# zeahmed/NeuralASR

Measured on AMD Instinct MI355X. Metric: audio-frames/sec (fwd+bwd+CTC+Adam) at batch 16 per GPU, higher is better.
Workload: dtype f32

## Files before the change

neuralasr_amd/csrc/nasr_api.hip:

```cpp
#include "nasr_ctx.h"

using namespace nasr;
using namespace nasr_impl;

namespace {
int settle_end(nasr_ctx* h, nasr_ctx::StepEnd& e, int* void_out) {
  if (!wait_stamp(e.stamp, e.seq, 60.0)) return h->fail(NASR_ERR_HIP, "nasr_settle_step: the step did not end within 60 s");
  if (*e.host != 0.f) {
    *void_out = 1;
    (void)rec_check(h);
  }
  return NASR_OK;
}
}

namespace nasr_impl {

int create_fail(nasr_ctx* h, int code, const std::string& m) {
  g_create_error = m;
  nasr_destroy(h);
  return code;
}

int handle_open(const char* fn, Family family, int device_id, void* stream, nasr_ctx** out, hipDeviceProp_t* prop) {
// ... 162 lines not shown
      for (int i = 0; i < h->ndense; ++i) {
        h->off_dftp[i] = df; df += tph_bytes(h->dWp[i], h->dIp[i]);
        h->off_dbtp[i] = db; if (i > 0 || h->npre == 0) db += tph_bytes(h->dIp[i], h->dWp[i]);
      }
      if (hipMalloc(h->WfTP.out(), of) != hipSuccess ||
          hipMalloc(h->WbTP.out(), std::max<size_t>(ob, 1024)) != hipSuccess ||
          hipMalloc(h->DfTP.out(), std::max<size_t>(df, 1024)) != hipSuccess ||
          hipMalloc(h->DbTP.out(), std::max<size_t>(db, 1024)) != hipSuccess)
        return create_fail(h, NASR_ERR_HIP, "hipMalloc of the tiled weight planes failed");
    }
  }
  const size_t ub = (size_t)h->L * h->D * h->Hp * h->N4 * 4;
  if (!alloc_param_buffers(h) || hipMalloc(h->Uf.out(), ub) != hipSuccess || hipMalloc(h->Ub.out(), ub) != hipSuccess)
    return create_fail(h, NASR_ERR_HIP, "hipMalloc of parameter buffers failed");
  {
    h->bucket_of_layer.assign(h->L, -1);
    if (h->L > 1 && h->L <= MAX_BUCKETS) {
      for (int l = h->L - 1; l >= 1; --l) {
        const int64_t lo = h->off_wx[l], hi = l == h->L - 1 ? h->np_int : h->off_wx[l + 1];
        h->bucket_of_layer[l] = (int)h->buckets.size();
        h->buckets.push_back({GRAD_HEAD + lo, hi - lo});
      }
      h->buckets.push_back({0, GRAD_HEAD + h->off_wx[1]});
    } else if (h->L == 1 && h->npre > 0) {
      h->bucket_of_layer[0] = 0;
      h->buckets.push_back({GRAD_HEAD + h->off_wx[0], h->np_int - h->off_wx[0]});
      h->buckets.push_back({0, GRAD_HEAD + h->off_wx[0]});
    } else {
      h->buckets.push_back({0, GRAD_HEAD + h->np_int});
    }
  }
  (void)hipMemsetAsync(h->Uf, 0, ub, h->st);
  (void)hipMemsetAsync(h->Ub, 0, ub, h->st);
  {
    const char* e = getenv("NASR_PERSIST");
    const char* er = getenv("NASR_REC");
    if (rec_setup(h, !(e && e[0] == '0') && prop.multiProcessorCount == 256, er && std::string(er) == "f32") != NASR_OK)
      return create_fail(h, NASR_ERR_HIP, t_err);
  }
  h->gates.resize(h->L);
  h->OTT.resize(h->L);
  h->ott_valid.assign(h->L, 0);
  h->outb.resize(h->L);
  h->cbuf.resize(h->L);
  h->Ybuf.resize(h->ndense);
  h->dYbuf.resize(h->ndense);
  if (int rc = handle_finish(h)) return rc;
  {
    const char* eo = getenv("NASR_WGRAD_OVERLAP");
    const bool eligible = h->rec_kind == RecKind::Persist && h->Hp == 512 && h->L > 1;
    h->wg_overlap = eligible && !(eo && eo[0] == '0');
    h->ev_wg.resize(h->L);
    h->wg_pending.assign(h->L, 0);
    if (eligible) {
      int lo = 0, hi = 0;
      (void)hipDeviceGetStreamPriorityRange(&lo, &hi);
      if (hipStreamCreateWithPriority(h->wst.out(), hipStreamNonBlocking, lo) != hipSuccess ||
          hipEventCreateWithFlags(h->ev_dx.out(), hipEventDisableTiming) != hipSuccess)
        return create_fail(h, NASR_ERR_HIP, "set-up of the weight-gradient side stream failed");
      for (auto& e : h->ev_wg)
        if (hipEventCreateWithFlags(e.out(), hipEventDisableTiming) != hipSuccess) return create_fail(h, NASR_ERR_HIP, "hipEventCreate failed");
      h->bwd_lean = true;
    }
  }
  if (h->rec_kind != RecKind::Step) {
    const char* er = getenv("NASR_PERSIST_REARM");
    h->rearm_after = er && *er ? std::max<long long>(0, atoll(er)) : 200;
  }
  if (h->rec_kind == RecKind::Persist) {
    const char* eb = getenv("NASR_BUCKET_DEFER");
    h->bucket_defer = !(eb && eb[0] == '0');
  }
  rec_start(h);
  *out = h;
  return NASR_OK;
}

int nasr_destroy(nasr_handle h) {
  if (!h) return NASR_OK;
  (void)hipSetDevice(h->device);
  for (const Stream* s : {&h->st, &h->cst, &h->d2h, &h->wst})
    if (*s) (void)hipStreamSynchronize(*s);
  (void)nasr_comm_destroy(h);
  drop_graphs(h);
  delete h;
  return NASR_OK;
}

const char* nasr_last_error(nasr_handle h) {
  if (!h) return g_create_error.c_str();
  return t_err_handle == h ? t_err.c_str() : "";
}
const char* nasr_backend(nasr_handle) { return "hip-gfx950"; }

int nasr_synchronize(nasr_handle h) {
  if (!h) return NASR_ERR_ARG;
  return sync_checked(h);
}

int64_t nasr_param_count(nasr_handle h) {
  MODEL_CALL(h);
  return h ? h->np_tf : -1;
}
int nasr_num_tensors(nasr_handle h) {
  MODEL_CALL(h);
  return h ? (int)h->tensors.size() : -1;
}

int nasr_tensor_info(nasr_handle h, int idx, char name[64], int64_t* offset, int64_t* rows, int64_t* cols) {
  MODEL_CALL(h);
  if (!h) return NASR_ERR_ARG;
  if (idx < 0 || idx >= (int)h->tensors.size()) return h->fail(NASR_ERR_ARG, "tensor index out of range");
  const TensorInfo& t = h->tensors[idx];
  if (name) {
    strncpy(name, t.name.c_str(), 63);
// ... 741 lines not shown
int nasr_get_phase_times(nasr_handle h, nasr_phase_times* out) {
  MODEL_CALL(h);
  if (!h || !out) return NASR_ERR_ARG;
  HIPCHK(h, hipStreamSynchronize(h->st));
  float acc[PH_COUNT] = {0};
  for (const auto& s : h->spans) {
    float ms = 0.f;
    if (hipEventElapsedTime(&ms, s.a, s.b) == hipSuccess) acc[s.ph] += ms;
  }
  nasr_phase_times t;
  memset(&t, 0, sizeof(t));
  t.pack_ms = acc[PH_PACK]; t.xproj_ms = acc[PH_XPROJ]; t.rec_fwd_ms = acc[PH_RECF]; t.proj_ctc_ms = acc[PH_PROJCTC];
  t.proj_bwd_ms = acc[PH_PROJB]; t.rec_bwd_ms = acc[PH_RECB]; t.wgrad_ms = acc[PH_WGRAD]; t.adam_ms = acc[PH_ADAM];
  float tot = 0.f;
  if (h->total_valid && hipEventElapsedTime(&tot, h->ev_total_a, h->ev_total_b) == hipSuccess) t.total_ms = tot;
  (void)hipGetLastError();
  t.rec_fwd_launches = h->n_fwd_launch;
  t.rec_bwd_launches = h->n_bwd_launch;
  *out = t;
  return NASR_OK;
}

int nasr_set_graph_mode(nasr_handle h, int enabled) {
  MODEL_CALL(h);
  if (!h) return NASR_ERR_ARG;
  h->graph_mode = enabled != 0;
  if (!h->graph_mode) drop_graphs(h);
  return NASR_OK;
}

int nasr_set_dropout_state(nasr_handle h, uint32_t seed, uint32_t counter) {
  MODEL_CALL(h);
  if (!h) return NASR_ERR_ARG;
  LSTM_CALL(h, "has no dropout");
  h->drop_seed = seed;
  h->drop_counter = counter;
  return NASR_OK;
}

int nasr_get_dropout_state(nasr_handle h, uint32_t* seed, uint32_t* counter) {
  MODEL_CALL(h);
  if (!h) return NASR_ERR_ARG;
  LSTM_CALL(h, "has no dropout");
  if (seed) *seed = h->drop_seed;
  if (counter) *counter = h->drop_counter;
  return NASR_OK;
}

int nasr_set_wgrad_overlap(nasr_handle h, int enabled) {
  MODEL_CALL(h);
  if (!h) return NASR_ERR_ARG;
  LSTM_CALL(h, "has no recurrence");
  if (enabled && !h->wst) return h->fail(NASR_ERR_STATE, "the weight-gradient side stream was not set up for this handle "
                                                         "(needs the persistent recurrence at Hp = 512 and more than one layer)");
  HIPCHK(h, hipStreamSynchronize(h->st));
  h->wg_overlap = enabled != 0;
  if (h->resident) return ensure_shape(h, h->B, h->T, h->Lmax);
  return NASR_OK;
}

int nasr_get_wgrad_overlap(nasr_handle h) {
  MODEL_CALL(h);
  return h && h->wg_overlap ? 1 : 0;
}

int nasr_set_bucket_defer(nasr_handle h, int defer) {
  MODEL_CALL(h);
  if (!h) return NASR_ERR_ARG;
  h->bucket_defer = defer != 0;
  return NASR_OK;
}

int nasr_get_persist_stats(nasr_handle h, int* aborts, int* rearms) {
  MODEL_CALL(h);
  if (!h) return NASR_ERR_ARG;
  if (aborts) *aborts = h->persist_aborts;
  if (rearms) *rearms = h->persist_rearms;
  return NASR_OK;
}

}
```

neuralasr_amd/csrc/nasr_batch.hip:

```cpp
#include "nasr_ctx.h"

using namespace nasr;
using namespace nasr_impl;

namespace nasr_impl {

int ensure_ctc_buffers(nasr_ctx* h, int B, int Bp, int T, int Tp, int Lmax, bool* grew) {
  const int KS = std::max(1, (2 * std::max(Lmax, 0) + 1 + 63) / 64);
  if (KS > 16) return h->fail(NASR_ERR_ARG, "label length > 511 not supported by the CTC lattice kernel");
  const int KSa = KS <= 1 ? 2 : KS <= 8 ? KS : (KS <= 12 ? 12 : 16);
  bool ok = true;
  ok &= h->logits.ensure((size_t)Tp * Bp * h->Cp * 4, grew);
  ok &= h->logz.ensure((size_t)Tp * Bp * 4, grew);
  ok &= h->alpha.ensure((size_t)B * (T + 8) * KSa * 64 * 4, grew);
  ok &= h->beta.ensure((size_t)B * (T + 8) * KSa * 64 * 4, grew);
  ok &= h->aoff.ensure((size_t)B * (T + 8) * 8, grew);
  ok &= h->boff.ensure((size_t)B * (T + 8) * 8, grew);
  ok &= h->logp.ensure((size_t)Bp * 8, grew);
  ok &= h->ctcprobs.ensure((size_t)Tp * Bp * h->Cp * 4, grew);
  ok &= h->ctckexp.ensure((size_t)B * 2 * ((T + 8) / 4 + 3) * 8, grew);
  ok &= h->nll.ensure((size_t)Bp * 4, grew);
  ok &= h->loss.ensure(16, grew);
  ok &= h->amax.ensure((size_t)Tp * Bp * 4, grew);
  ok &= h->ids.ensure((size_t)B * Tp * 4, grew);
// ... 13 lines not shown
  const size_t R = (size_t)T * Bp;
  const int D = h->D, Hp = h->Hp, N4 = h->N4;
  bool grew = false;
  bool ok = true;
  const int KSa = ensure_ctc_buffers(h, B, Bp, T, Tp, Lmax, &grew);
  if (KSa < 0) return KSa;
  ok &= h->X0.ensure(R * h->Fp * 4, &grew);
  ok &= h->seqbuf.ensure((size_t)Bp * 4, &grew);
  ok &= h->dout.ensure(R * D * Hp * 4, &grew);
  ok &= h->hstate.ensure((size_t)2 * D * Bp * Hp * 4, &grew);
  ok &= h->partial.ensure((size_t)2 * D * (Hp / 32) * Bp * Hp * 4, &grew);
  ok &= h->dcstate.ensure((size_t)2 * D * Bp * Hp * 4, &grew);
  ok &= h->dgbuf.ensure(R * D * N4 * 4, &grew);
  if (h->rec_kind == RecKind::Persist) ok &= h->dgmax.ensure(persist_dgmax_floats(T, Bp, Hp, D) * 4, &grew);
  {
    int ipmax = h->Fp, wmax = D * N4;
    for (int l = 0; l < h->L; ++l) ipmax = std::max(ipmax, h->Ip[l]);
    for (int i = 0; i < h->ndense; ++i) { ipmax = std::max(ipmax, h->dIp[i]); wmax = std::max(wmax, h->dWp[i]); }
    ok &= h->XTP.ensure(tph_bytes((int)R, ipmax), &grew);
    ok &= h->X0TTP.ensure(tph_bytes(h->Ip[0], (int)R), &grew);
    for (int l = 0; l < h->L; ++l) ok &= h->OTT[l].ensure(tph_bytes(D * Hp, (int)R), &grew);
    ok &= h->GTP.ensure(tph_bytes((int)R, wmax), &grew);
    ok &= h->GTTP.ensure(tph_bytes(wmax, (int)R), &grew);
    if (h->wg_overlap) {
      ok &= h->GTTP2.ensure(tph_bytes(wmax, (int)R), &grew);
      ok &= h->sc_gc2.ensure((size_t)wmax);
    }
    if (h->ndense) ok &= h->DTP.ensure(tph_bytes(ipmax, (int)R), &grew);
    {
      const size_t n15 = std::max<size_t>(R, (size_t)std::max(ipmax, wmax));
      if (n15 > h->sc15_n) {
        ok &= h->sc15.ensure(n15);
        if (ok) {
          launch_fill(h->sc15.sp(), 32768.f, (int)n15, h->st);
          launch_fill(h->sc15.ip(), 1.f / 32768.f, (int)n15, h->st);
          h->sc15_n = n15;
        }
      }
      ok &= h->sc_x0r.ensure(R) && h->sc_x0c.ensure((size_t)h->Fp);
      ok &= h->sc_gr.ensure(R) && h->sc_gc.ensure((size_t)wmax);
      if (h->compactable) {
        ok &= h->sc_cr.ensure(R + 64) && h->sc_cx.ensure(R + 64);
        ok &= h->OTS.ensure((h->wg_overlap ? 2 : 1) * tph_bytes(D * Hp, (int)R), &grew);
      }
      for (int i = 0; i < h->ndense; ++i) ok &= h->sc_yr[i].ensure(R) && h->sc_yc[i].ensure((size_t)h->dWp[i]);
      bool g2 = false;
      ok &= h->scws.ensure(tph_scale_ws_floats((int)R, std::max(ipmax, wmax)) * 4, &g2);
    }
  }
  int csw = std::max(D * N4, h->Cp);
  for (int i = 0; i < h->ndense; ++i) csw = std::max(csw, h->dWp[i]);
  ok &= h->csws.ensure((size_t)std::max(32, tp_split2_parts((int)R)) * csw * 4, &grew);
  if (h->wg_overlap) ok &= h->csws2.ensure((size_t)std::max(32, tp_split2_parts((int)R)) * csw * 4, &grew);
  for (int i = 0; i < h->ndense; ++i) {
    ok &= h->Ybuf[i].ensure(R * h->dWp[i] * 4, &grew);
    ok &= h->dYbuf[i].ensure(R * h->dWp[i] * 4, &grew);
  }
  for (int l = 0; l < h->L; ++l) {
    ok &= h->gates[l].ensure(R * D * N4 * 4, &grew);
    ok &= h->outb[l].ensure(R * D * Hp * 4, &grew);
    ok &= h->cbuf[l].ensure(R * D * Hp * 4, &grew);
  }
  if (!ok) return h->fail(NASR_ERR_HIP, "hipMalloc failed while sizing batch buffers");
  if (grew || Bp != h->Bp) drop_graphs(h);
  h->B = B; h->Bp = Bp; h->T = T; h->Lmax = Lmax; h->Tp = Tp; h->KS = KSa;
  return NASR_OK;
}

int validate_batch(nasr_ctx* h, const int32_t* seq_len, const int32_t* labels, const int32_t* label_len, int B, int T,
                   int Lmax, int num_classes) {
  const bool las = !num_classes && h->family == Family::Las;
  const int C = num_classes ? num_classes : h->C;
  if (B < 1 || B > 64) return h->fail(NASR_ERR_ARG, "per-GPU batch must be in [1,64]");
  if (T < 1) return h->fail(NASR_ERR_ARG, "T must be >= 1");
  for (int b = 0; b < B; ++b) {
    if (seq_len[b] < 1 || seq_len[b] > T)
      return h->fail(NASR_ERR_ARG, "seq_len[" + std::to_string(b) + "] out of [1,T]");
    if (!labels) continue;
    if (las) {
      if (label_len[b] < 0 || label_len[b] > Lmax)
        return h->fail(NASR_ERR_ARG, "label_len[" + std::to_string(b) + "] out of [0,Lmax]");
      for (int i = 0; i < Lmax; ++i) {
        const int v = labels[(size_t)b * Lmax + i];
        if (v < 0 || v >= C) return h->fail(NASR_ERR_ARG, "label id out of [0, num_classes-1]");
      }
      continue;
    }
    const int L = label_len[b];
    if (L < 0 || L > Lmax) return h->fail(NASR_ERR_ARG, "label_len[" + std::to_string(b) + "] out of [0,Lmax]");
    int rep = 0;
    for (int i = 0; i < L; ++i) {
      const int v = labels[(size_t)b * Lmax + i];
      if (v < 0 || v >= C - 1)
        return h->fail(NASR_ERR_ARG, "label id out of [0, num_classes-2] (blank = num_classes-1 is not a label)");
      if (i > 0 && v == labels[(size_t)b * Lmax + i - 1]) ++rep;
    }
    if (L + rep > seq_len[b])
      return h->fail(NASR_ERR_INFEASIBLE, "Not enough time for target transition sequence (required: " +
                                              std::to_string(L + rep) + ", available: " + std::to_string(seq_len[b]) +
                                              ") in sequence " + std::to_string(b));
  }
  return NASR_OK;
}

int validate_chunk(nasr_ctx* h, const int32_t* n_frames, int S, int Tc) {
  if (Tc < 1) return h->fail(NASR_ERR_ARG, "a stream chunk needs Tc >= 1");
// ... 306 lines not shown
```

neuralasr_amd/csrc/nasr_ctx.h:

```cpp
#pragma once
#include <hip/hip_runtime.h>

#include <dlfcn.h>
#include <sched.h>
#include <unistd.h>

#include <chrono>

#include <algorithm>
#include <cmath>
#include <cstdio>
#include <cstdlib>
#include <cstring>
#include <functional>
#include <map>
#include <memory>
#include <mutex>
#include <string>
#include <vector>

#include "../../include/nasr.h"
#include "kernels.h"
#include "resample.h"
#include "wave_aug.h"
// ... 250 lines not shown
  DevBuf scws;
  int gttp_layer = -1;
  int dgmax_layer = -1;
  DevBuf dgmax;
  DevPtr<float> Gbase;
  std::vector<std::pair<int64_t, int64_t>> buckets;
  std::vector<Event> ev_bucket;
  std::vector<int> bucket_of_layer;
  bool bucket_defer = true;
  DevPtr<AdamDev> adam_dev;
  float lr;
  float max_grad_norm = 0.f;
  DevPtr<ClipDev> clip_dev;
  DevPtr<double> clip_part;
  struct StepRes { Pinned<void> host; size_t cap = 0; Pinned<uint32_t> stamp; uint32_t seq = 0; bool valid = false; int B = 0, Bp = 0, Tp = 0; bool logits = false, greedy = false;
                   Event ev_lg; };
  StepRes res[2];
  int res_cur = 0;
  struct StepEnd { Pinned<float> host; uint32_t* stamp = nullptr; uint32_t seq = 0; bool valid = false; int64_t token = 0; };
  static constexpr int NEND = 4;
  StepEnd endw[NEND];
  int end_cur = 0;
  int64_t step_token = 0;
  uint32_t stamp_seq = 0;

  bool resident = false, have_grads = false, have_fwd = false;
  int B = 0, Bp = 0, T = 0, Lmax = 0, Tp = 0, KS = 1;
  int64_t frames = 0;
  std::vector<int32_t> h_seq;
  BatchSlot slots[NSLOT];
  BatchSlot* cur = nullptr;
  Stream cst;
  Stream d2h;
  Event ev_snap;
  DevBuf logits_snap;
  std::mutex slot_mu;
  int slot_rr = 0;
  int32_t *seq_p = nullptr, *lablen_p = nullptr, *labels_p = nullptr, *cstart_p = nullptr, *cpos_p = nullptr,
          *rowmap_p = nullptr;
  bool compactable = false;
  int cmp_rows = 0, cmp_rows_p = 0;
  int32_t *vrow_p = nullptr, *vprev_p = nullptr, *vnext_p = nullptr;
  SV sc_cr, sc_cx;
  DevBuf OTS;

  bool wg_overlap = false;
  bool bwd_lean = false;
  Stream wst;
  Event ev_dx;
  std::vector<Event> ev_wg;
  std::vector<char> wg_pending;
  DevBuf GTTP2, csws2, slabs2;
  SV sc_gc2;
  DevBuf XTP, X0TTP, GTP, GTTP;
  std::vector<DevBuf> OTT;
  std::vector<char> ott_valid;
  DevBuf ctcprobs, ctckexp;
  DevBuf seqbuf, X0, logits, logz, alpha, beta, aoff, boff, logp, nll, loss, slabs, csws, amax, ids, lens,
      stage;
  DevBuf al_logz, al_bp, al_path, al_score, al_logits, al_meta;
  std::vector<DevBuf> gates, outb, cbuf;
  DevBuf dout, hstate, partial, dcstate, dgbuf;

  bool graph_mode = true;
  bool step_decode = false, step_logits = false, have_decoded = false;
  bool step_greedy = false;
  std::map<GraphKey, hipGraphExec_t> graphs;

  bool profiling = false;
  std::vector<Event> ev_pool;
  size_t ev_used = 0;
  struct Span { int ph; hipEvent_t a, b; };
  std::vector<Span> spans;
  Event ev_total_a, ev_total_b;
  bool window_open = false, total_valid = false;
  int n_fwd_launch = 0, n_bwd_launch = 0;
  nasr_phase_times last_times;

  int fail(int code, const std::string& m) {
    t_err = m;
    t_err_handle = this;
    return code;
  }
};

namespace nasr_impl {

#define HIPCHK(h, expr)                                                                                   \
  do {                                                                                                    \
    hipError_t e_ = (expr);                                                                               \
    if (e_ != hipSuccess)                                                                                 \
      return (h)->fail(NASR_ERR_HIP, std::string(#expr) + ": " + hipGetErrorString(e_));                  \
  } while (0)
#define MODEL_CALL(h)                                                                                     \
  do {                                                                                                    \
    if ((h) && (h)->family == Family::Featurizer)                                                         \
      return (h)->fail(NASR_ERR_STATE, std::string(__func__) + ": a featurizer handle has no model");     \
  } while (0)
#define LSTM_CALL(h, reason)                                                                              \
  do {                                                                                                    \
    if ((h) && (h)->family != Family::Lstm)                                                               \
      return (h)->fail(NASR_ERR_STATE, std::string(__func__) + ": a WaveNet or LAS handle " reason);      \
  } while (0)
#define FAMILY_CALL(h, state, text)                                                                       \
  do {                                                                                                    \
    if (!(h)) return NASR_ERR_ARG;                                                                        \
// ... 118 lines not shown
  bool rs = false;
  int n = 0;
  std::vector<int64_t> uoff, foff;
  int64_t S_in = 0;
  size_t mb = 0, meta_bytes = 0, rmeta_bytes = 0;
  bool wave = false;
  WavePlan wp;
};
int fz_plan(nasr_ctx* eh, FzState& z, const std::string& fn, const int64_t* offsets, const int32_t* rates, int n, FzPlan* p);
int fz_wave_plan(nasr_ctx* eh, FzState& z, const std::string& fn, const nasr_wave_aug* wave, FzPlan* p);
size_t fz_stage_bytes(const FzPlan& p);
int fz_produce_slot(nasr_ctx* eh, nasr_ctx* fzh, const FzPlan& p, const float* audio, int Tb, float* dcentre, float* dpad,
                    void* pinned, hipStream_t st);
int fz_feature_width(const nasr_ctx* fzh, int* numcontext, int* frame_width);
int fz_static_width(const nasr_ctx* fzh);

struct FzFeedSlot {
  int64_t seg_off, ntail, in_off, nnew;
  int64_t keep_off, nkeep;
  int64_t lead;
  int64_t f_off, nfb, want;
  int64_t nnorm, upto, y_off;
  int64_t T;
  int64_t rows0, nrows;
  int64_t n_after;
};
struct FzFeedPlan {
  std::vector<FzFeedSlot> slot;
  int64_t seg_total = 0, in_total = 0, f_total = 0, y_total = 0;
  int Tc = 0;
};
int fz_stream_attach(nasr_ctx* eh, nasr_ctx* fzh, int S, std::unique_ptr<FzStream, FzStreamDelete>* out);
int fz_stream_plan(nasr_ctx* eh, const FzStream& a, const std::string& fn, const int64_t* nnew, const uint8_t* last, FzFeedPlan* p);
int fz_stream_run(nasr_ctx* eh, FzStream& a, const FzFeedPlan& p, const float* audio, float* dfeats, hipStream_t st);
void fz_stream_advance(FzStream& a, const FzFeedPlan& p, const uint8_t* last);
void fz_stream_reset(FzStream& a, int slot);

inline float* dout_of(nasr_ctx* h, int) { return h->dout.as<float>(); }
inline float* dg_of(nasr_ctx* h, int) { return h->dgbuf.as<float>(); }
inline bool wg_alt(const nasr_ctx* h, int l) { return h->wg_overlap && (l & 1); }
inline unsigned char* gttp_of(nasr_ctx* h, int l) { return (wg_alt(h, l) ? h->GTTP2 : h->GTTP).as<unsigned char>(); }
inline float* csws_of(nasr_ctx* h, int l) { return (wg_alt(h, l) ? h->csws2 : h->csws).as<float>(); }
inline nasr_ctx::SV& gc_of(nasr_ctx* h, int l) { return wg_alt(h, l) ? h->sc_gc2 : h->sc_gc; }
inline const float* lstm_input(nasr_ctx* h, int l) {
  if (l > 0) return h->outb[l - 1].as<float>();
  return h->npre ? h->Ybuf[h->npre - 1].as<float>() : h->X0.as<float>();
}

int gemm_f32(nasr_ctx* h, GemmDesc g);
int gemm_dense(nasr_ctx* h, const float* A, const float* B, float* C, int M, int N, int K, int lda, int ldb, int ldc, bool a_col,
               bool b_col, const float* bias = nullptr, int a_shift = 0, int a_rows = -1);
inline float* fp(const DevBuf& b, size_t off = 0) { return b.as<float>() + off; }
int forward(nasr_ctx* h, bool chunk = false);
int loss_pass(nasr_ctx* h, bool training);
CtcDims ctc_dims(nasr_ctx* h);
int ctc_forward(nasr_ctx* h);
int backward(nasr_ctx* h);
int fetch_logits(nasr_ctx* h, float* logits_out, int rows = -1);

int wn_ensure_shape(nasr_ctx* h, int B, int T, int Lmax);
int wn_forward(nasr_ctx* h, bool training);
int wn_backward(nasr_ctx* h);

int las_ensure_shape(nasr_ctx* h, int B, int T, int Lmax);
int las_forward(nasr_ctx* h, bool sample);
int las_backward(nasr_ctx* h);

}
```

neuralasr_amd/csrc/nasr_layout.hip:

```cpp
#include "nasr_ctx.h"

using namespace nasr;
using namespace nasr_impl;

namespace nasr_impl {

std::string g_create_error;
thread_local std::string t_err;
thread_local const void* t_err_handle = nullptr;

void pl_scales(nasr_ctx* h, const float* src, int rows, int K, int ld, nasr_ctx::SV* row, nasr_ctx::SV* col, hipStream_t st) {
  launch_tph_scales(src, rows, K, ld, row ? row->sp() : nullptr, row ? row->ip() : nullptr, col ? col->sp() : nullptr,
                    col ? col->ip() : nullptr, h->scws.as<float>(), st);
}
void pl_split(const float* src, unsigned char* tpN, unsigned char* tpT, int rows, int K, int ld, const float* rs,
              const float* cs, float* colpart, hipStream_t st) {
  launch_tph_split2(src, tpN, tpT, rows, K, ld, rs, 1.f, cs, 1.f, colpart, st);
}
void pl_gemm(GemmTPHDesc g, const float* a_inv, const float* b_inv, hipStream_t st, int64_t ainv_bstride, int64_t binv_bstride) {
  g.a_inv = a_inv; g.b_inv = b_inv; g.ainv_bstride = ainv_bstride; g.binv_bstride = binv_bstride;
  launch_gemm_tph(g, st);
}
__global__ void stamp_kernel(unsigned* dst, unsigned value, float* f0_dst, const float* f0_src) {
  if (f0_dst) __hip_atomic_store(f0_dst, *f0_src, __ATOMIC_RELAXED, __HIP_MEMORY_SCOPE_SYSTEM);
  __hip_atomic_store(dst, value, __ATOMIC_RELEASE, __HIP_MEMORY_SCOPE_SYSTEM);
}
void launch_stamp(unsigned* dst, unsigned value, float* f0_dst, const float* f0_src, hipStream_t st) {
  hipLaunchKernelGGL(stamp_kernel, dim3(1), dim3(1), 0, st, dst, value, f0_dst, f0_src);
}

__global__ __launch_bounds__(256) void publish_results_kernel(const float* __restrict__ loss, const float* __restrict__ fault,
                                                              const int* __restrict__ lens, int Bp, const int* __restrict__ ids,
                                                              int n_ids, unsigned* host, unsigned* stamp, unsigned value) {
  if (threadIdx.x == 0) {
    host[0] = __float_as_uint(*loss);
    host[1] = __float_as_uint(*fault);
  }
  for (int i = threadIdx.x; i < Bp; i += 256) host[2 + i] = (unsigned)lens[i];
  for (int i = threadIdx.x; i < n_ids; i += 256) host[2 + Bp + i] = (unsigned)ids[i];
  __threadfence_system();
  __syncthreads();
  if (threadIdx.x == 0) __hip_atomic_store(stamp, value, __ATOMIC_RELEASE, __HIP_MEMORY_SCOPE_SYSTEM);
}
void launch_publish_results(const float* loss, const float* fault, const int* lens, int Bp, const int* ids, int n_ids, void* host,
                            unsigned* stamp, unsigned value, hipStream_t st) {
  hipLaunchKernelGGL(publish_results_kernel, dim3(1), dim3(256), 0, st, loss, fault, lens, Bp, ids, n_ids,
                     static_cast<unsigned*>(host), stamp, value);
}

bool wait_stamp(const uint32_t* w, uint32_t want, double timeout_s) {
  const volatile uint32_t* v = w;
  for (int i = 0; i < 4000; ++i)
    if (*v == want) return true;
  const auto t0 = std::chrono::steady_clock::now();
  for (unsigned n = 0;; ++n) {
    if (*v == want) return true;
    if ((n & 63) == 63) {
      if (std::chrono::duration<double>(std::chrono::steady_clock::now() - t0).count() > timeout_s) return false;
      usleep(20);
    } else {
      sched_yield();
    }
  }
}

int sync_checked(nasr_ctx* h) {
  HIPCHK(h, hipStreamSynchronize(h->st));
  return rec_check(h);
}

void drop_graphs(nasr_ctx* h) {
  for (auto& kv : h->graphs) (void)hipGraphExecDestroy(kv.second);
  h->graphs.clear();
}

hipEvent_t next_event(nasr_ctx* h) {
  if (h->ev_used == h->ev_pool.size()) (void)hipEventCreate(h->ev_pool.emplace_back().out());
  return h->ev_pool[h->ev_used++];
}
int build_layout(nasr_ctx* h) {
  const nasr_model_cfg& c = h->cfg;
  h->F = c.feature_size;
  h->H = c.hidden;
  h->L = c.num_layers;
  h->D = c.bidirectional ? 2 : 1;
  h->C = c.num_classes;
  h->Fp = rup(h->F, 32);
  h->Hp = rup(h->H, 64);
  h->N4 = 4 * h->Hp;
  h->Cp = rup(h->C, 32);
  const bool concat = c.bidirectional && c.merge == NASR_MERGE_CONCAT;
  const int D = h->D, Hp = h->Hp, N4 = h->N4, H = h->H;
  const int lstm_out = concat ? 2 * H : H, lstm_outp = concat ? 2 * Hp : Hp;

  h->npre = c.num_pre;
  h->has_post = c.post_width > 0;
  h->ndense = h->npre + (h->has_post ? 1 : 0);
  h->dWid.assign(h->ndense, 0); h->dWp.assign(h->ndense, 0); h->dIn.assign(h->ndense, 0); h->dIp.assign(h->ndense, 0);
  for (int i = 0; i < h->npre; ++i) {
    h->dWid[i] = c.pre_width[i]; h->dWp[i] = rup(c.pre_width[i], 64);
    h->dIn[i] = i == 0 ? h->F : h->dWid[i - 1];
    h->dIp[i] = i == 0 ? h->Fp : h->dWp[i - 1];
  }
  if (h->has_post) {
    const int i = h->npre;
    h->dWid[i] = c.post_width; h->dWp[i] = rup(c.post_width, 64);
    h->dIn[i] = lstm_out; h->dIp[i] = lstm_outp;
  }
  h->F0 = h->npre ? h->dWid[h->npre - 1] : h->F;
  h->Pin = h->has_post ? c.post_width : lstm_out;
  h->Pinp = h->has_post ? h->dWp[h->npre] : lstm_outp;

  int64_t off = 0;
  h->off_dw.assign(h->ndense, 0); h->off_db.assign(h->ndense, 0);
  for (int i = 0; i < h->ndense; ++i) {
    h->off_dw[i] = off; off += (int64_t)h->dIp[i] * h->dWp[i];
    h->off_db[i] = off; off += h->dWp[i];
  }
  h->Ip.resize(h->L);
  h->off_wx.resize(h->L);
// ... 163 lines not shown
```

neuralasr_amd/csrc/nasr_pass.hip:

```cpp
#include "nasr_ctx.h"

using namespace nasr;
using namespace nasr_impl;

namespace nasr_impl {

int run_steps(nasr_ctx* h, int l, bool bwd, int s0, int s1, hipStream_t st, int* launches) {
  if (h->rec_use != RecKind::Step && s0 == 0 && s1 == h->T) return rec_launch(h, l, bwd, st, launches);
  *launches += s1 - s0;
  const LstmDims dm{h->T, h->B, h->Bp, h->H, h->Hp, h->D};
  const size_t sU = (size_t)l * h->D * h->Hp * h->N4;
  const size_t hs = (size_t)h->D * h->Bp * h->Hp;
  const size_t ps = (size_t)h->D * lstm_bwd_partials(h->Hp) * h->Bp * h->Hp;
  float* hst = h->hstate.as<float>();
  float* par = h->partial.as<float>();
  float* dcs = h->dcstate.as<float>();
  auto body = [&]() {
    if (!bwd) {
      if (s0 == 0) (void)hipMemsetAsync(hst, 0, hs * 4, st);
      for (int s = s0; s < s1; ++s)
        launch_lstm_fwd_step(dm, s, h->Uf + sU, hst + (s & 1) * hs, hst + ((s + 1) & 1) * hs,
                             h->gates[l].as<float>(), h->cbuf[l].as<float>(), h->outb[l].as<float>(),
                             h->seq_p, h->cfg.forget_bias, st);
    } else {
// ... 143 lines not shown
  {
    GemmTPHDesc g{};
    g.A = h->DTP.as<unsigned char>(); g.B = h->GTTP.as<unsigned char>(); g.C = h->G + h->off_dw[i];
    g.M = Ip; g.N = Wp; g.K = R; g.nkbA = nkb; g.nkbB = nkb; g.ldc = Wp;
    g.split_k = gemm_tph_pick_split(g.M, g.N, g.K);
    g.slabs = ensure_slabs(h, g.split_k, g.M, g.N);
    if (g.split_k > 1 && !g.slabs) return h->fail(NASR_ERR_HIP, "slab workspace allocation failed");
    pl_gemm(g, as.cinv, h->sc_gc.ip(), h->st);
  }
  launch_colsum_parts(h->csws.as<float>(), tp_split2_parts(R), Wp, h->G + h->off_db[i], h->st);
  if (dX) {
    GemmTPHDesc g{};
    g.A = h->GTP.as<unsigned char>(); g.B = h->DbTP + h->off_dbtp[i]; g.C = dX;
    g.M = R; g.N = Ip; g.K = Wp; g.nkbA = (Wp + 15) / 16; g.nkbB = g.nkbA; g.ldc = Ip;
    g.split_k = gemm_tph_pick_split(g.M, g.N, g.K);
    g.slabs = ensure_slabs(h, g.split_k, g.M, g.N);
    if (g.split_k > 1 && !g.slabs) g.split_k = 1;
    pl_gemm(g, h->sc_gr.ip(), h->sc_dr[i].ip(), h->st);
  }
  HIPCHK(h, hipGetLastError());
  return NASR_OK;
}

static int run_chunk_steps(nasr_ctx* h, int l, hipStream_t st) {
  StreamState& ss = *h->stream;
  const LstmDims dm{h->T, h->B, h->Bp, h->H, h->Hp, h->D};
  const size_t sU = (size_t)l * h->D * h->Hp * h->N4, hs = (size_t)h->D * h->Bp * h->Hp;
  float* hst = h->hstate.as<float>();
  float* state = ss.state.as<float>() + (size_t)l * ss.S * 2 * h->H;
  float *g = h->gates[l].as<float>(), *c = h->cbuf[l].as<float>(), *o = h->outb[l].as<float>();
  if (ss.la) launch_la_load_state(state, hst, ss.cimg.as<float>(), ss.S, h->H, h->Bp, h->Hp, st);
  else launch_stream_load_state(state, hst, ss.cimg.as<float>(), ss.S, h->H, h->Bp, h->Hp, st);
  launch_lstm_fwd_step_carry(dm, h->Uf + sU, hst, hst + hs, g, c, o, h->seq_p, h->cfg.forget_bias, ss.cimg.as<float>(), st);
  for (int s = 1; s < h->T; ++s)
    launch_lstm_fwd_step(dm, s, h->Uf + sU, hst + (s & 1) * hs, hst + ((s + 1) & 1) * hs, g, c, o, h->seq_p, h->cfg.forget_bias, st);
  if (ss.la) launch_la_save_state(o, c, ss.la->sl, state, ss.S, h->H, h->Bp, h->Hp, st);
  else launch_stream_save_state(o, c, h->seq_p, state, ss.S, h->H, h->Bp, h->Hp, st);
  h->n_fwd_launch += h->T;
  HIPCHK(h, hipGetLastError());
  return NASR_OK;
}

int forward(nasr_ctx* h, bool chunk) {
  if (!h->resident) return h->fail(NASR_ERR_STATE, "no resident batch: call nasr_upload_batch first");
  switch (h->family) {
    case Family::WaveNet: return wn_forward(h, false);
    case Family::Las: return h->fail(NASR_ERR_STATE, "a LAS handle has no CTC logits: use nasr_las_forward");
    default: break;
  }
  const int Bp = h->Bp, T = h->T, D = h->D, Hp = h->Hp;
  const int R = T * Bp;
  h->n_fwd_launch = 0;
  std::fill(h->ott_valid.begin(), h->ott_valid.end(), 0);
  if (!chunk) HIPCHK(h, hipMemsetAsync(h->Gbase, 0, GRAD_HEAD * 4, h->st));
  if (h->rec_use == RecKind::Persist && !chunk) {
    HIPCHK(h, hipMemsetAsync(h->pctl + 1, 0, (size_t)h->L * sizeof(PersistCtl), h->st));
    HIPCHK(h, hipMemsetAsync(h->xchf, 0, (size_t)h->L * persist_hx_bytes(h->Hp), h->st));
  }
  for (int i = 0; i < h->npre; ++i) {
    PhaseScope ps(h, PH_XPROJ);
    int rc = dense_forward(h, i, i == 0 ? h->X0.as<float>() : h->Ybuf[i - 1].as<float>());
    if (rc) return rc;
  }
  for (int l = 0; l < h->L; ++l) {
    {
      PhaseScope ps(h, PH_XPROJ);
      gemm_xproj(h, l, R, h->st);
      HIPCHK(h, hipGetLastError());
    }
    PhaseScope ps(h, PH_RECF);
    int rc = chunk ? run_chunk_steps(h, l, h->st) : run_steps(h, l, false, 0, T, h->st, &h->n_fwd_launch);
    if (rc) return rc;
  }
  if (h->has_post) {
    PhaseScope ps(h, PH_XPROJ);
    int rc = dense_forward(h, h->npre, h->outb[h->L - 1].as<float>());
    if (rc) return rc;
  }
  if (h->ndense && !chunk) h->drop_counter += 1;
  {
    PhaseScope ps(h, PH_PROJCTC);
    const bool sr = h->cfg.merge == NASR_MERGE_STACK_RESHAPE && D == 2;
    GemmDesc g{};
    g.A = h->has_post ? h->Ybuf[h->npre].as<float>() : h->outb[h->L - 1].as<float>();
    g.B = h->P + h->off_w;
    g.C = h->logits.as<float>();
    g.M = h->Tp * Bp; g.N = h->Cp; g.K = h->Pinp;
    g.lda = sr ? Hp : h->Pinp; g.ldb = h->Cp; g.ldc = h->Cp;
    g.a_map = sr ? h->rowmap_p : nullptr;
    g.a_rows = sr ? 2 * R : R;
    g.bias = h->P + h->off_b;
    g.split_k = gemm_pick_split(g.M, g.N, g.K);
    if (int rc = gemm_f32(h, g)) return rc;
  }
  h->have_fwd = !chunk;
  return NASR_OK;
}

CtcDims ctc_dims(nasr_ctx* h) {
  CtcDims d;
  d.Tp = h->Tp; d.B = h->B; d.Bp = h->Bp; d.C = h->C; d.Cp = h->Cp; d.Lmax = std::max(h->Lmax, 1);
  d.KS = h->KS; d.Tws = h->T + 8;
  d.lprobs = h->ctcprobs.as<float>(); d.goff = h->ctckexp.as<double>();
  return d;
}

// ... 69 lines not shown
    dg_scales(h, l, R, false, ws);
    launch_tph_split2(dG, nullptr, GT, rows, D * N4, D * N4, nullptr, 1.f, gc.sp(), 1.f, cs_part, ws, vm);
  }
  h->gttp_layer = -1;
  const ActScale ao = act_out(h), ai = lstm_in_scale(h, l);
  for (int m = std::max(l - 1, 0); m <= (vm ? l - 1 : l); ++m)
    if (!h->ott_valid[m]) {
      launch_tph_split2(h->outb[m].as<float>(), nullptr, h->OTT[m].as<unsigned char>(), rows, D * Hp, D * Hp, nullptr, 1.f, ao.cs, 1.f,
                        nullptr, ws, vm);
      h->ott_valid[m] = 1;
    }
  unsigned char* OS = h->OTS.as<unsigned char>() + (wg_alt(h, l) ? tph_bytes(D * Hp, R) : 0);
  if (vm)
    launch_tph_split2(h->outb[l].as<float>(), nullptr, OS, rows, D * Hp, D * Hp, nullptr, 1.f, ao.cs, 1.f, nullptr, ws, h->vprev_p,
                      D == 2 ? h->vnext_p : nullptr, Hp);
  if (l == 0 && h->npre)
    pl_split(lstm_input(h, l), nullptr, h->X0TTP.as<unsigned char>(), R, h->Ip[0], h->Ip[0], nullptr, ai.cs, nullptr, ws);
  {
    GemmTPHDesc g{};
    g.A = l == 0 ? h->X0TTP.as<unsigned char>() : h->OTT[l - 1].as<unsigned char>();
    g.B = GT; g.C = h->G + h->off_wx[l];
    g.M = h->Ip[l]; g.N = D * N4; g.K = rows; g.nkbA = nkb; g.nkbB = nkb; g.ldc = D * N4;
    g.side = side;
    g.split_k = gemm_tph_pick_split(g.M, g.N, g.K);
    g.slabs = slabs_for(g.split_k, g.M, g.N);
    if (g.split_k > 1 && !g.slabs) return h->fail(NASR_ERR_HIP, "slab workspace allocation failed");
    pl_gemm(g, ai.cinv, gc.ip(), ws);
  }
  launch_colsum_parts(cs_part, tp_split2_parts(rows), D * N4, h->G + h->off_bias[l], ws);
  {
    GemmTPHDesc g{};
    g.A = vm ? OS : h->OTT[l].as<unsigned char>(); g.B = GT; g.C = h->G + h->off_u[(size_t)l * D];
    g.M = Hp; g.N = N4; g.K = rows; g.nkbA = nkb; g.nkbB = nkb; g.ldc = N4;
    g.a_kshift = vm ? 0 : -Bp;
    g.nbatch = D;
    g.a_bstride = (size_t)(Hp / 32) * pl_rb_bytes(nkb); g.b_bstride = (size_t)(N4 / 32) * pl_rb_bytes(nkb);
    g.c_bstride = (int64_t)Hp * N4;
    g.a_kshift1 = vm ? 0 : Bp;
    g.side = side;
    g.split_k = gemm_tph_pick_split(g.M, g.N, g.K, D);
    g.slabs = slabs_for(g.split_k * D, g.M, g.N);
    if (g.split_k > 1 && !g.slabs) return h->fail(NASR_ERR_HIP, "slab workspace allocation failed");
    pl_gemm(g, ao.cinv, gc.ip(), ws, Hp, N4);
  }
  HIPCHK(h, hipGetLastError());
  return NASR_OK;
}

int wg_join(nasr_ctx* h, int l) {
  if (l >= 0 && l < h->L && h->wg_pending[l]) {
    HIPCHK(h, hipStreamWaitEvent(h->st, h->ev_wg[l], 0));
    h->wg_pending[l] = 0;
  }
  return NASR_OK;
}

int backward(nasr_ctx* h) {
  switch (h->family) {
    case Family::WaveNet: return wn_backward(h);
    case Family::Las: return las_backward(h);
    default: break;
  }
  const int Bp = h->Bp, T = h->T, D = h->D, Hp = h->Hp;
  const int R = T * Bp, Rp = h->Tp * Bp;
  const bool sr = h->cfg.merge == NASR_MERGE_STACK_RESHAPE && D == 2;
  if (h->rec_use == RecKind::Persist) {
    HIPCHK(h, hipMemsetAsync(h->pctl + 1 + h->L, 0, (size_t)h->L * sizeof(PersistCtl), h->st));
    HIPCHK(h, hipMemsetAsync(h->xchb, 0, (size_t)h->L * persist_px_bytes(), h->st));
  }
  {
    PhaseScope ps(h, PH_PROJCTC);
    const CtcDims d = ctc_dims(h);
    launch_ctc_grad(d, h->logits.as<float>(), h->logz.as<float>(), h->lablen_p, h->seq_p,
                    h->cstart_p, h->cpos_p, h->alpha.as<float>(), h->beta.as<float>(),
                    h->aoff.as<double>(), h->boff.as<double>(), h->logp.as<double>(), 1.f / (float)h->B, h->st);
    HIPCHK(h, hipGetLastError());
  }
  {
    PhaseScope ps(h, PH_PROJB);
    GemmDesc g{};
    g.A = h->has_post ? h->Ybuf[h->npre].as<float>() : h->outb[h->L - 1].as<float>();
    g.B = h->logits.as<float>();
    g.C = h->G + h->off_w;
    g.M = h->Pinp; g.N = h->Cp; g.K = Rp;
    g.lda = sr ? Hp : h->Pinp; g.ldb = h->Cp; g.ldc = h->Cp;
    g.a_col = true; g.a_map = sr ? h->rowmap_p : nullptr; g.a_rows = sr ? 2 * R : R;
    g.split_k = gemm_pick_split(g.M, g.N, g.K);
    if (int rc = gemm_f32(h, g)) return rc;
    launch_colsum(h->logits.as<float>(), Rp, h->Cp, h->Cp, h->G + h->off_b, h->csws.as<float>(), h->st);
    GemmDesc x{};
    x.A = h->logits.as<float>();
    x.B = h->P + h->off_w;
    x.C = h->has_post ? h->dYbuf[h->npre].as<float>() : dout_of(h, h->L - 1);
    x.M = Rp; x.N = h->Pinp; x.K = h->Cp;
    x.lda = h->Cp; x.ldb = h->Cp; x.ldc = sr ? Hp : h->Pinp;
    x.b_col = true; x.a_rows = Rp; x.c_map = sr ? h->rowmap_p : nullptr; x.split_k = 1;
    if (int rc = gemm_f32(h, x)) return rc;
  }
  if (h->has_post) {
    PhaseScope ps(h, PH_WGRAD);
    int rc = dense_backward(h, h->npre, h->outb[h->L - 1].as<float>(), dout_of(h, h->L - 1));
    if (rc) return rc;
  }
  h->n_bwd_launch = 0;
  h->dgmax_layer = -1;
  for (int l = h->L - 1; l >= 0; --l) {
    const bool defer = h->rec_use != RecKind::Step && h->bucket_defer;
    {
      PhaseScope ps(h, PH_RECB);
      int rc = run_steps(h, l, true, 0, T, h->st, &h->n_bwd_launch);
      if (rc) return rc;
    }
    if (defer && l + 1 < h->L && h->bucket_of_layer[l + 1] >= 0) {
      if (int rc = wg_join(h, l + 1)) return rc;
      HIPCHK(h, hipEventRecord(h->ev_bucket[h->bucket_of_layer[l + 1]], h->st));
    }
    PhaseScope ps(h, PH_WGRAD);
    if (int rc = wg_join(h, l + 2)) return rc;
    if (l > 0 || h->npre > 0) gemm_dx(h, l, R, h->st);
    const bool side = h->wg_overlap && h->rec_use == RecKind::Persist && l > 0 && h->gttp_layer == l;
    if (side) {
      HIPCHK(h, hipEventRecord(h->ev_dx, h->st));
      HIPCHK(h, hipStreamWaitEvent(h->wst, h->ev_dx, 0));
      int rc = weight_grads(h, l, h->wst, true);
      if (rc) return rc;
      HIPCHK(h, hipEventRecord(h->ev_wg[l], h->wst));
      h->wg_pending[l] = 1;
    } else {
      int rc = weight_grads(h, l, h->st, false);
      if (rc) return rc;
    }
    if (h->bucket_of_layer[l] >= 0 && !(defer && l > 0)) {
      if (int rc = wg_join(h, l)) return rc;
      HIPCHK(h, hipEventRecord(h->ev_bucket[h->bucket_of_layer[l]], h->st));
    }
  }
  for (int l = 0; l < h->L; ++l)
    if (int rc = wg_join(h, l)) return rc;
  for (int i = h->npre - 1; i >= 0; --i) {
    PhaseScope ps(h, PH_WGRAD);
    int rc = dense_backward(h, i, i == 0 ? h->X0.as<float>() : h->Ybuf[i - 1].as<float>(),
                            i > 0 ? h->dYbuf[i - 1].as<float>() : nullptr);
// ... 22 lines not shown
```

Baseline: 1.206 million.

## Move output-projection weight-gradient GEMM and bias colsum to side stream

In the persistent-recurrence backward pass, the output-projection weight-gradient GEMM and its bias column sum now run on the low-priority weight-gradient stream, so they overlap with the input-gradient GEMM and the recurrent backward. An event joins the work back before the last layer's gradients are consumed and at the start of the next forward. The change also adds a separate colsum workspace and slab buffer, and synchronises the side stream in the checked-sync and overlap-toggle paths. It costs extra events and memory and adds a risk of contention or ordering hazards on shared buffers such as the logits.

```diff
diff --git a/neuralasr_amd/csrc/nasr_api.hip b/neuralasr_amd/csrc/nasr_api.hip
--- a/neuralasr_amd/csrc/nasr_api.hip
+++ b/neuralasr_amd/csrc/nasr_api.hip
@@ -238,15 +238,16 @@
     h->wg_overlap = eligible && !(eo && eo[0] == '0');
     h->ev_wg.resize(h->L);
     h->wg_pending.assign(h->L, 0);
-    if (eligible) {
+    if (h->rec_kind == RecKind::Persist) {
       int lo = 0, hi = 0;
       (void)hipDeviceGetStreamPriorityRange(&lo, &hi);
-      if (hipStreamCreateWithPriority(h->wst.out(), hipStreamNonBlocking, lo) != hipSuccess ||
-          hipEventCreateWithFlags(h->ev_dx.out(), hipEventDisableTiming) != hipSuccess)
+      if (hipStreamCreateWithPriority(h->wst.out(), hipStreamNonBlocking, lo) != hipSuccess)
         return create_fail(h, NASR_ERR_HIP, "set-up of the weight-gradient side stream failed");
+      for (Event* e : {&h->ev_dx, &h->ev_proj})
+        if (hipEventCreateWithFlags(e->out(), hipEventDisableTiming) != hipSuccess) return create_fail(h, NASR_ERR_HIP, "hipEventCreate failed");
       for (auto& e : h->ev_wg)
         if (hipEventCreateWithFlags(e.out(), hipEventDisableTiming) != hipSuccess) return create_fail(h, NASR_ERR_HIP, "hipEventCreate failed");
-      h->bwd_lean = true;
+      h->bwd_lean = eligible;
     }
   }
   if (h->rec_kind != RecKind::Step) {
@@ -1094,8 +1095,9 @@
   if (!h) return NASR_ERR_ARG;
   LSTM_CALL(h, "has no recurrence");
   if (enabled && !h->wst) return h->fail(NASR_ERR_STATE, "the weight-gradient side stream was not set up for this handle "
-                                                         "(needs the persistent recurrence at Hp = 512 and more than one layer)");
+                                                         "(needs the persistent recurrence)");
   HIPCHK(h, hipStreamSynchronize(h->st));
+  if (h->wst) HIPCHK(h, hipStreamSynchronize(h->wst));
   h->wg_overlap = enabled != 0;
   if (h->resident) return ensure_shape(h, h->B, h->T, h->Lmax);
   return NASR_OK;
diff --git a/neuralasr_amd/csrc/nasr_batch.hip b/neuralasr_amd/csrc/nasr_batch.hip
--- a/neuralasr_amd/csrc/nasr_batch.hip
+++ b/neuralasr_amd/csrc/nasr_batch.hip
@@ -89,6 +89,7 @@
   for (int i = 0; i < h->ndense; ++i) csw = std::max(csw, h->dWp[i]);
   ok &= h->csws.ensure((size_t)std::max(32, tp_split2_parts((int)R)) * csw * 4, &grew);
   if (h->wg_overlap) ok &= h->csws2.ensure((size_t)std::max(32, tp_split2_parts((int)R)) * csw * 4, &grew);
+  if (h->wg_overlap) ok &= h->csws3.ensure((size_t)32 * h->Cp * 4, &grew);
   for (int i = 0; i < h->ndense; ++i) {
     ok &= h->Ybuf[i].ensure(R * h->dWp[i] * 4, &grew);
     ok &= h->dYbuf[i].ensure(R * h->dWp[i] * 4, &grew);
diff --git a/neuralasr_amd/csrc/nasr_ctx.h b/neuralasr_amd/csrc/nasr_ctx.h
--- a/neuralasr_amd/csrc/nasr_ctx.h
+++ b/neuralasr_amd/csrc/nasr_ctx.h
@@ -326,6 +326,9 @@
   std::vector<char> wg_pending;
   DevBuf GTTP2, csws2, slabs2;
   SV sc_gc2;
+  Event ev_proj;
+  bool proj_pending = false;
+  DevBuf csws3;
   DevBuf XTP, X0TTP, GTP, GTTP;
   std::vector<DevBuf> OTT;
   std::vector<char> ott_valid;
@@ -550,6 +553,7 @@
                bool b_col, const float* bias = nullptr, int a_shift = 0, int a_rows = -1);
 inline float* fp(const DevBuf& b, size_t off = 0) { return b.as<float>() + off; }
 int forward(nasr_ctx* h, bool chunk = false);
+int wg_join(nasr_ctx* h, int l);
 int loss_pass(nasr_ctx* h, bool training);
 CtcDims ctc_dims(nasr_ctx* h);
 int ctc_forward(nasr_ctx* h);
diff --git a/neuralasr_amd/csrc/nasr_layout.hip b/neuralasr_amd/csrc/nasr_layout.hip
--- a/neuralasr_amd/csrc/nasr_layout.hip
+++ b/neuralasr_amd/csrc/nasr_layout.hip
@@ -66,6 +66,7 @@
 
 int sync_checked(nasr_ctx* h) {
   HIPCHK(h, hipStreamSynchronize(h->st));
+  if (h->wst) HIPCHK(h, hipStreamSynchronize(h->wst));
   return rec_check(h);
 }
 
diff --git a/neuralasr_amd/csrc/nasr_pass.hip b/neuralasr_amd/csrc/nasr_pass.hip
--- a/neuralasr_amd/csrc/nasr_pass.hip
+++ b/neuralasr_amd/csrc/nasr_pass.hip
@@ -219,6 +219,8 @@
   const int R = T * Bp;
   h->n_fwd_launch = 0;
   std::fill(h->ott_valid.begin(), h->ott_valid.end(), 0);
+  for (int l = 0; l < h->L; ++l)
+    if (int rc = wg_join(h, l)) return rc;
   if (!chunk) HIPCHK(h, hipMemsetAsync(h->Gbase, 0, GRAD_HEAD * 4, h->st));
   if (h->rec_use == RecKind::Persist && !chunk) {
     HIPCHK(h, hipMemsetAsync(h->pctl + 1, 0, (size_t)h->L * sizeof(PersistCtl), h->st));
@@ -394,6 +396,10 @@
     HIPCHK(h, hipStreamWaitEvent(h->st, h->ev_wg[l], 0));
     h->wg_pending[l] = 0;
   }
+  if (l == h->L - 1 && h->proj_pending) {
+    HIPCHK(h, hipStreamWaitEvent(h->st, h->ev_proj, 0));
+    h->proj_pending = false;
+  }
   return NASR_OK;
 }
 
@@ -410,6 +416,7 @@
     HIPCHK(h, hipMemsetAsync(h->pctl + 1 + h->L, 0, (size_t)h->L * sizeof(PersistCtl), h->st));
     HIPCHK(h, hipMemsetAsync(h->xchb, 0, (size_t)h->L * persist_px_bytes(), h->st));
   }
+  const bool pside = h->wg_overlap && h->rec_use == RecKind::Persist;
   {
     PhaseScope ps(h, PH_PROJCTC);
     const CtcDims d = ctc_dims(h);
@@ -428,8 +435,21 @@
     g.lda = sr ? Hp : h->Pinp; g.ldb = h->Cp; g.ldc = h->Cp;
     g.a_col = true; g.a_map = sr ? h->rowmap_p : nullptr; g.a_rows = sr ? 2 * R : R;
     g.split_k = gemm_pick_split(g.M, g.N, g.K);
-    if (int rc = gemm_f32(h, g)) return rc;
-    launch_colsum(h->logits.as<float>(), Rp, h->Cp, h->Cp, h->G + h->off_b, h->csws.as<float>(), h->st);
+    if (pside) {
+      bool grew = false;
+      if (g.split_k > 1 && !h->slabs2.ensure((size_t)g.split_k * g.M * g.N * 4, &grew))
+        return h->fail(NASR_ERR_HIP, "slab workspace allocation failed");
+      g.slabs = g.split_k > 1 ? h->slabs2.as<float>() : nullptr;
+      HIPCHK(h, hipEventRecord(h->ev_dx, h->st));
+      HIPCHK(h, hipStreamWaitEvent(h->wst, h->ev_dx, 0));
+      launch_gemm(g, h->wst);
+      launch_colsum(h->logits.as<float>(), Rp, h->Cp, h->Cp, h->G + h->off_b, h->csws3.as<float>(), h->wst);
+      HIPCHK(h, hipEventRecord(h->ev_proj, h->wst));
+      h->proj_pending = true;
+    } else {
+      if (int rc = gemm_f32(h, g)) return rc;
+      launch_colsum(h->logits.as<float>(), Rp, h->Cp, h->Cp, h->G + h->off_b, h->csws.as<float>(), h->st);
+    }
     GemmDesc x{};
     x.A = h->logits.as<float>();
     x.B = h->P + h->off_w;
```

Result: no change. 1.212 million, median of 6 (+0.6%).
